# bnbowman/pbccs

Hardware: AMD Instinct MI355X
Metric: CCS ZMWs/sec (and GCUPS) at 1/2/4/8 MI355X vs host-CPU ccs (higher is better)
Workload: dtype f64

## Files before the change

### include/pbccs_amd.h

```cpp
#ifndef PBCCS_AMD_H
#define PBCCS_AMD_H

#ifdef __cplusplus
extern "C" {
#endif

#define PBCCS_OK 0
#define PBCCS_EINVAL (-1)
#define PBCCS_EOOM (-2)
#define PBCCS_EDEVICE (-3)
#define PBCCS_ESTATE (-4)
#define PBCCS_ERANGE (-5)

#define PBCCS_INSERTION 0
#define PBCCS_DELETION 1
#define PBCCS_SUBSTITUTION 2
#define PBCCS_FORWARD_STRAND 0
#define PBCCS_REVERSE_STRAND 1
#define PBCCS_ADD_SUCCESS 0
#define PBCCS_ADD_ALPHABETAMISMATCH 1
#define PBCCS_ADD_MEM_FAIL 2
#define PBCCS_ADD_POOR_ZSCORE 3
#define PBCCS_ADD_OTHER 4
#define PBCCS_ZMW_SUCCESS 0
// ... 118 lines not shown
    long long fill_launches, score_launches, score_tasks, mutations;
    long long band_top_bytes;
    long long band_region_bytes;
    long long band_used_bytes;
    long long pool_mapped_bytes;
    long long oom_retries;
    long long create_host_ns;
    long long create_upload_ns;
    long long derive_ns;
    long long fill_work[16];
    long long scan_reads;
    long long uncertain_reads;
    long long exact_rounds;
    long long uncertain_why[4];
    long long repeat_skipped_ckpt;
} pbccs_counters;
int pbccs_engine_counters(pbccs_engine* eng, pbccs_counters* out, int reset);

typedef struct {
    char name[32];
    long long launches;
    double device_ms;
    double cells;
    double bytes;
    double wave_s;
} pbccs_kernel_stat;
int pbccs_engine_set_profiling(pbccs_engine* eng, int on);
int pbccs_engine_kernel_stats(pbccs_engine* eng, pbccs_kernel_stat* out, int cap, int* n, int reset);


// ... 710 lines not shown
```

### pbccs_amd/csrc/arrow_device.hpp

```cpp
#pragma once

#include <hip/hip_runtime.h>
#include <stdint.h>

namespace pbccs {

constexpr int kCtxZero = 8;
constexpr int kCtxStride = 5;
constexpr int kNoMutation = -100;
constexpr int kMaxExtCols = 4;
constexpr int kMaxFlipFlops = 5;
constexpr double kAlphaBetaTol = 0.001;
constexpr double kRebandFrac = 0.04;

enum MutType : int { kIns = 0, kDel = 1, kSub = 2 };
enum Strand : int { kFwd = 0, kRev = 1 };

enum FillStatus : int { kFillOk = 0, kFillMismatch = 1, kFillOverflow = 2, kFillBadInput = 3, kFillTall = 4,
                        kFillUncertain = 5 };
constexpr double kUnitRoundoff = 0x1p-53;

__host__ __device__ inline int mut_code(int pos, int type, int base) { return (pos << 4) | (type << 2) | base; }
__host__ __device__ inline int mut_pos(int c) { return c >> 4; }
__host__ __device__ inline int mut_type(int c) { return (c >> 2) & 3; }
// ... 23 lines not shown
    const long long* rSeqOff;
    const int* rLen;
    const int* rStrand;
    const int* rTs;
    const int* rTe;
    const int* rActive;
    const int* rZmw;
    const long long* rColBase;
    const long long* rValA;
    const long long* rValB;
    const long long* rValCap;
    const int* rCkpt;
    const char* seqPool;
    int2* aRange;
    int* aOff;
    double* aLs;
    double* aPre;
    int2* bRange;
    int* bOff;
    double* bLs;
    double* bSuf;
    double* valPool;
    double* rBaseline;
    double* rDev;
    int* rFlips;
    int* rStatus;
    double prNot;
    double prThird;
    double sdn;
    unsigned long long* stats;
};

enum StatKind : int { kStatFill = 0, kStatSuffix = 1, kStatScore = 2, kStatFillTall = 3 };
enum WaveSlot : int { kWaveFill = 10, kWaveFillTall = 11, kWaveScore = 12, kWaveSuffix = 13, kWaveReduce = 14 };
#ifndef PBCCS_WAVE_STAMPS
#define PBCCS_WAVE_STAMPS 0
#endif
__device__ __forceinline__ long long wave_t0(const unsigned long long* stats)
{
    if (!PBCCS_WAVE_STAMPS) return 0;
    return stats ? (long long)__builtin_amdgcn_s_memrealtime() : 0;
}
__device__ __forceinline__ void wave_ticks(unsigned long long* stats, int slot, long long t0)
{
    if (!PBCCS_WAVE_STAMPS || !stats) return;
// ... 419 lines not shown
```

### pbccs_amd/csrc/arrow_kernels.hip

```cpp
#include "arrow_device.hpp"
#include "arrow_kernels.hpp"
#include "arrow_score_device.hpp"
#include "coop_chain.hpp"

#include <climits>

namespace pbccs {

__device__ __forceinline__ LaneBand scratch_band(const FillScratch& F, int g, int l, int which)
{
    const long long gm = 2LL * g + which;
    LaneBand m;
    m.range = F.range + gm * F.capCols * 64 + l;
    m.off = F.off + gm * F.capCols * 64 + l;
    m.ls = F.ls + gm * F.capCols * 64 + l;
    m.val = F.val + gm * F.capSlots * 64 + l;
    m.cap = F.capSlots;
    return m;
}

__global__ void __launch_bounds__(64) k_fill(DevBatch B, FillScratch F, const int* __restrict__ reads, int n)
{
    const int t = blockIdx.x * blockDim.x + threadIdx.x;
    if (t >= n) return;
// ... 180 lines not shown
        }
        __syncthreads();
    }
}

constexpr int kSuffixTile = 2048;

__device__ __forceinline__ double add8(double s, const double* __restrict__ t)
{
    double v[8];
#pragma unroll
    for (int i = 0; i < 8; ++i) v[i] = t[i];
#pragma unroll
    for (int i = 0; i < 8; ++i) s = s + v[i];
    return s;
}

__device__ __forceinline__ void k_suffix_body(DevBatch B, const int* __restrict__ reads, int n, int withPrefix)
{
    __shared__ double tile[kSuffixTile];
    const int r = reads[blockIdx.x];
    if (B.rStatus[r] != kFillOk && B.rStatus[r] != kFillMismatch) return;
    const long long cb = B.rColBase[r];
    const int J = window_view(B, r).Length();
    const double* ls = B.bLs + cb;
    double* suf = B.bSuf + cb;
    const int ncol = J + 1;
    const int lane = threadIdx.x & 63;
    const int wbase = threadIdx.x & ~63;
    for (int k0 = 0; k0 <= ncol; k0 += blockDim.x) {
// ... 4 lines not shown
            __syncthreads();
            for (int q = threadIdx.x; q < kSuffixTile && c0 + q < ncol; q += blockDim.x) tile[q] = ls[c0 + q];
            __syncthreads();
            const int hi = min(ncol - c0, kSuffixTile);
            int q = max(kb - c0, 0);
            const int headEnd = min(hi, kb + 64 - c0);
            for (; q < headEnd; ++q) {
                const double v = tile[q];
                if (c0 + q >= k) s = s + v;
            }
            for (; q + 8 <= hi; q += 8) s = add8(s, tile + q);
            for (; q < hi; ++q) s = s + tile[q];
        }
        if (k <= ncol) suf[k] = s;
    }
    if (!withPrefix) return;
    if (threadIdx.x != 0) return;
    const double* als = B.aLs + cb;
    double* pre = B.aPre + cb;
    double run = 0.0;
    pre[0] = 0.0;
    int k = 0;
    for (; k + 8 <= ncol; k += 8) {
        double v[8];
#pragma unroll
        for (int q = 0; q < 8; ++q) v[q] = als[k + q];
#pragma unroll
        for (int q = 0; q < 8; ++q) {
            run = run + v[q];
            pre[k + q + 1] = run;
// ... 74 lines not shown

__device__ __forceinline__ MidGeom middle_geometry(const Band& a, const Band& b, int sc, int bc)
{
    MidGeom g;
    const int2 r0 = a.range[sc - 1], r1 = a.range[sc], r2 = a.range[sc + 1], r3 = a.range[sc + 2];
    g.b0 = min(min(r1.x, r0.x), r2.x);
    g.e0 = max(max(r1.y, r0.y), r2.y);
    g.b1 = min(min(r2.x, r1.x), r3.x);
    g.e1 = max(max(r2.y, r1.y), r3.y);
    const int2 q0 = b.range[bc], q1 = b.range[bc + 1];
    g.lb = min(min(g.b0, g.b1), min(q0.x, q1.x));
    g.le = max(max(g.e0, g.e1), max(q0.y, q1.y));
    return g;
}

__device__ __forceinline__ double score_middle(const ScoreCtx& S, int sc, int bc, const MidGeom& g,
                                               const double* __restrict__ av, int2 ar,
                                               const double* __restrict__ bv, int2 br,
                                               const char* __restrict__ rdp, TaskStat& st)
{
    const int I = S.I;
    char t0, t1, t2, t3;
    int x0, x1, x2, x3;
    S.tv.At(sc - 2, t0, x0);
    S.tv.At(sc - 1, t1, x1);
    S.tv.At(sc, t2, x2);
    S.tv.At(sc + 1, t3, x3);
    (void)t0;
    const double* P0 = S.P.P(sc > 1 ? x0 : kCtxZero);
    const double* P1 = S.P.P(x1);
    const double* P2 = S.P.P(x2);
    const double pM0 = P0[kM], pD0 = P0[kD], cB0 = P1[kB], cS0 = P1[kS3];
    const double pM1 = P1[kM], pD1 = P1[kD], cB1 = P2[kB], cS1 = P2[kS3];
    const double lM = P2[kM], lD = P2[kD];
    const double pn = S.P.prNot, p3 = S.P.prThird;

#define PB_ALPHA(i) (((i) >= ar.x && (i) < ar.y) ? av[(i)] : 0.0)
#define PB_BETA(i) (((i) >= br.x && (i) < br.y) ? bv[-(i)] : 0.0)
#define PB_CELL(out, i, rb, curB, nxtB, pM, pD, cB, cS, pd, pl, rawPrev)                    \
    {                                                                                     \
        const double em_ = ((rb) == (curB)) ? pn : p3;                                    \
        double s_ = ((i) > 0) ? (((i) < I) ? (pd) * (pM) * em_ : 0.0) : (rawPrev);        \
        if ((i) > 1 && (i) < I) s_ = s_ + (rawPrev) * (((nxtB) == (rb)) ? (cB) : (cS));   \
        if ((i) != I) s_ = s_ + (pl) * (pD);                                              \
        out = s_;                                                                         \
    }

    double C0 = 0.0;
    {
        double aD = PB_ALPHA(g.b0 - 1), raw = 0.0;
        for (int i = g.b0; i < g.e0; ++i) {
            const double aL = PB_ALPHA(i);
            const char rb = rdp[i - 1];
            double v;
            PB_CELL(v, i, rb, t1, t2, pM0, pD0, cB0, cS0, aD, aL, raw);
            raw = v;
            if (C0 < v) C0 = v;
            aD = aL;
        }
    }
    const bool s0 = (C0 != 0.0 && C0 != 1.0);
    const int u0 = min(g.b0, g.b1), u1 = max(g.e0, g.e1);
    double C1 = 0.0;
    {
        double aD = PB_ALPHA(u0 - 1), raw0 = 0.0, raw1 = 0.0, sc0p = 0.0;
        for (int i = u0; i < u1; ++i) {
            const double aL = PB_ALPHA(i);
            const char rb = rdp[i - 1];
            double v0 = 0.0, v1 = 0.0, sc0 = 0.0;
            if (i >= g.b0 && i < g.e0) {
                PB_CELL(v0, i, rb, t1, t2, pM0, pD0, cB0, cS0, aD, aL, raw0);
                sc0 = s0 ? v0 / C0 : v0;
            }
            if (i >= g.b1 && i < g.e1) {
                PB_CELL(v1, i, rb, t2, t3, pM1, pD1, cB1, cS1, sc0p, sc0, raw1);
                if (C1 < v1) C1 = v1;
            }
            raw0 = v0;
            raw1 = v1;
            sc0p = sc0;
            aD = aL;
        }
    }
    const bool s1 = (C1 != 0.0 && C1 != 1.0);
    double v = 0.0;
    {
        double aD = PB_ALPHA(g.lb - 1), raw0 = 0.0, raw1 = 0.0, sc0p = 0.0;
        double bH = PB_BETA(g.lb);
        for (int i = g.lb; i < g.le; ++i) {
            const double aL = PB_ALPHA(i);
            const double bN = PB_BETA(i + 1);
            const char rb = (i >= 1) ? rdp[i - 1] : (char)0;
            double v0 = 0.0, v1 = 0.0, sc0 = 0.0, sc1 = 0.0;
            if (i >= g.b0 && i < g.e0) {
                PB_CELL(v0, i, rb, t1, t2, pM0, pD0, cB0, cS0, aD, aL, raw0);
                sc0 = s0 ? v0 / C0 : v0;
            }
            if (i >= g.b1 && i < g.e1) {
                PB_CELL(v1, i, rb, t2, t3, pM1, pD1, cB1, cS1, sc0p, sc0, raw1);
                sc1 = s1 ? v1 / C1 : v1;
            }
            if (i < I) {
                const double mprob = lM * ((rdp[i] == t3) ? pn : p3);
                v = v + sc1 * mprob * bN;
// ... 204 lines not shown
            for (int q = lane; q < spanR; q += 64) ws.rd[q] = gr[q];
            aBase = offLo;
            bBase = boHi;
            rBase = r0;
        }
    }
    __syncthreads();

    TaskStat st;
    double d = 0.0;
    if (scored) {
        if (middle) {
            const int2 ar = S.a.range[sc - 1];
            const int2 br = S.b.range[bc];
            const int ao = S.a.off[sc - 1], bo = S.b.off[bc];
            double score;
            if (staged) {
                const double* av = ws.a + (ao - aBase) - ar.x;
                const double* bv = ws.b + (bo - bBase) + (br.y - 1);
                const char* rdp = ws.rd - rBase;
                score = score_middle(S, sc, bc, g, av, ar, bv, br, rdp, st);
            } else {
                const double* av = S.a.val + ao - ar.x;
                const double* bv = S.b.val + bo + (br.y - 1);
                score = score_middle(S, sc, bc, g, av, ar, bv, br, S.rd, st);
            }
            d = score - B.rBaseline[r];
        } else {
            const int slot = atomicAdd(W.edgeCount, 1);
            if (slot < W.edgeCap) {
                W.edgeList[3 * slot + 0] = k;
                W.edgeList[3 * slot + 1] = rr;
                W.edgeList[3 * slot + 2] = m;
            } else {
                atomicOr(scratch.overflow, 2);
            }
        }
    }
    if (valid && !(scored && !middle)) W.delta[W.deltaBase[k] + (long long)rr * M + m] = d;
    if (B.stats) {
// ... 314 lines not shown
                const double* src = bV + bO[ckB];
                for (int i = lane; i < r0.y - r0.x; i += 64) slot[sOff[nA] + i] = src[i];
                for (int j = ckB - 1; j >= jbLo; --j) {
                    const int2 nr = bR[j + 1], rg = bR[j];
                    __builtin_amdgcn_fence(__ATOMIC_ACQ_REL, "workgroup");
                    replay_beta(X, j, slot + sOff[nA + (ckB - (j + 1))], nr.x, nr.y, slot + sOff[nA + (ckB - j)], rg.x,
                                rg.y);
                }
            }
            __builtin_amdgcn_fence(__ATOMIC_ACQ_REL, "workgroup");
            if (mine) {
                const int2 ar = aR[ja];
                const int2 br = bR[bc];
                const double* av = slot + sOff[ja - ckA] - ar.x;
                const double* bv = slot + sOff[nA + (ckB - bc)] + (br.y - 1);
                const double score = score_middle(S, sc, bc, g, av, ar, bv, br, S.rd, st);
                W.delta[W.deltaBase[k] + (long long)rr * M + m] = score - B.rBaseline[r];
            }
            pending = pending && !mine;
            __syncthreads();
        }
        if (B.stats) {
            unsigned long long c2 = st.cells, b2 = st.bytes;
            for (int w = 32; w > 0; w >>= 1) {
                c2 += __shfl_xor(c2, w, 64);
                b2 += __shfl_xor(b2, w, 64);
            }
            if (lane == 0) {
                atomicAdd(&B.stats[2 * kStatScore], c2);
                atomicAdd(&B.stats[2 * kStatScore + 1], b2);
            }
// ... 325 lines not shown
```

### pbccs_amd/csrc/capi.hip

```cpp
#include "../../include/pbccs_amd.h"

#include <hip/hip_runtime.h>

#include <algorithm>
#include <array>
#include <atomic>
#include <chrono>
#include <cmath>
#include <condition_variable>
#include <cstdio>
#include <cstdlib>
#include <cstring>
#include <functional>
#include <limits>
#include <memory>
#include <mutex>
#include <new>
#include <stdexcept>
#include <string>
#include <thread>
#include <vector>

#include "align_band.hpp"
#include "align_kernels.hpp"
// ... 294 lines not shown
    out->band_region_bytes = eng->counters.bandRegionBytes;
    out->band_used_bytes = eng->counters.bandUsedBytes;
    long long mapped = 0;
    for (const auto& s : eng->slots) mapped += (long long)s->val.mapped_bytes();
    out->pool_mapped_bytes = mapped;
    out->oom_retries = eng->oomRetries;
    out->create_host_ns = eng->createHostNs;
    out->create_upload_ns = eng->createUploadNs;
    out->derive_ns = eng->counters.deriveNs;
    for (int k = 0; k < 16; ++k) out->fill_work[k] = eng->counters.fillWork[k];
    out->scan_reads = eng->counters.scanReads;
    out->uncertain_reads = eng->counters.uncertainReads;
    out->exact_rounds = eng->counters.exactRounds;
    for (int k = 0; k < 4; ++k) out->uncertain_why[k] = eng->counters.uncertainWhy[k];
    out->repeat_skipped_ckpt = eng->repeatSkippedCkpt;
    if (reset) {
        eng->counters = Counters();
        eng->oomRetries = 0;
        eng->repeatSkippedCkpt = 0;
        eng->createHostNs = eng->createUploadNs = 0;
    }
    return PBCCS_OK;
}

int pbccs_scorer_create(pbccs_engine* eng, const pbccs_arrow_config* cfg, const char* tpl, int tpl_len,
                        pbccs_scorer** out)
{
    if (!eng || !cfg || !tpl || tpl_len <= 0 || !out) return fail(PBCCS_EINVAL, "bad argument");
    return guarded([&] {
        std::unique_ptr<pbccs_scorer> s(new pbccs_scorer());
// ... 4 lines not shown
        *out = s.release();
        return PBCCS_OK;
    });
}

void pbccs_scorer_destroy(pbccs_scorer* s) { delete s; }

int pbccs_scorer_add_read(pbccs_scorer* s, const char* seq, int len, int strand, int tstart, int tend,
                          double threshold, int* result)
{
    if (!s || !seq || len < 0 || !result || (strand != 0 && strand != 1)) return fail(PBCCS_EINVAL, "bad argument");
    return guarded([&] {
        ArrowBatch& B = *s->batch;
        const int r = B.AppendRead(s->z, std::string(seq, len), strand, tstart, tend);
        B.FillReads({r});
        *result = B.FinishAddRead(r, threshold);
        return PBCCS_OK;
    });
}

int pbccs_scorer_score_many(pbccs_scorer* s, const pbccs_mutation* m, int n, double fast_threshold, double* scores)
{
    if (!s || (n > 0 && (!m || !scores)) || n < 0) return fail(PBCCS_EINVAL, "bad argument");
    return guarded([&] {
        ArrowBatch& B = *s->batch;
        const int L = (int)B.Template(s->z).size();
        std::vector<std::vector<int>> codes(1);
        for (int i = 0; i < n; ++i) {
            Mutation mu;
            if (!to_mutation(m[i], L, &mu)) return fail(PBCCS_EINVAL, "invalid single-base mutation");
// ... 207 lines not shown
static void merge_engine_stats(pbccs_engine* eng, ArrowBatch& B)
{
    std::lock_guard<std::mutex> lk(eng->statsMu);
    try {
        const Counters& c = B.counters();
        eng->counters.fillLaunches += c.fillLaunches;
        eng->counters.scoreLaunches += c.scoreLaunches;
        eng->counters.scoreTasks += c.scoreTasks;
        eng->counters.mutations += c.mutations;
        eng->counters.deriveNs += c.deriveNs;
        eng->counters.scanReads += c.scanReads;
        eng->counters.uncertainReads += c.uncertainReads;
        eng->counters.exactRounds += c.exactRounds;
        for (int k = 0; k < 4; ++k) eng->counters.uncertainWhy[k] += c.uncertainWhy[k];
        for (int k = 0; k < 16; ++k) eng->counters.fillWork[k] += c.fillWork[k];
        eng->counters.bandTopBytes = std::max(eng->counters.bandTopBytes, c.bandTopBytes);
        eng->counters.bandRegionBytes = std::max(eng->counters.bandRegionBytes, c.bandRegionBytes);
        eng->counters.bandUsedBytes = std::max(eng->counters.bandUsedBytes, c.bandUsedBytes);
        B.ResetCounters();
        B.CollectProfile(eng->stats);
    } catch (...) {
        (void)hipGetLastError();
    }
}

static int create_batch(pbccs_engine* eng, const pbccs_zmw_input* in, int n, const pbccs_polish_options* opts,
                        int slot, pbccs_batch** out, const pbccs_repeat_options* repeats = nullptr)
{
    if (!eng || n < 0 || (n > 0 && !in) || !out) return fail(PBCCS_EINVAL, "bad argument");
    return guarded([&] {
// ... 4286 lines not shown
```

### pbccs_amd/csrc/engine.hip

```cpp
#include "engine.hpp"
#include "diploid_kernels.hpp"
#include "refine_repeats.hpp"
#include "strand_kernels.hpp"

#include <hipcub/hipcub.hpp>

#include <algorithm>
#include <mutex>
#include <climits>
#include <cmath>
#include <cstdio>
#include <cstdlib>
#include <cstring>
#include <numeric>
#include <set>
#include <stdexcept>
#include <chrono>
#include <unordered_set>

namespace pbccs {

#define PBCCS_HIP(x)                                                         \
    do {                                                                     \
        hipError_t e_ = (x);                                                 \
// ... 316 lines not shown
{
    if (stream) (void)hipStreamSynchronize(stream);
    if (stream2) (void)hipStreamSynchronize(stream2);
    for (hipEvent_t e : eventPool) (void)hipEventDestroy(e);
    if (evFork) (void)hipEventDestroy(evFork);
    if (evJoin) (void)hipEventDestroy(evJoin);
    if (stream2) (void)hipStreamDestroy(stream2);
    if (stream) (void)hipStreamDestroy(stream);
}

size_t Workspace::TrimRetired()
{
    size_t b = 0;
    auto t = [&](auto& v) { b += v.trim(); };
    t(hDesc);
    t(selBase); t(nSel); t(colScratch); t(bump); t(desc); t(seq); t(ckPairs); t(ckStart); t(rBaseline); t(rFlips);
    t(rDev); t(wDev); t(wAmb);
    t(rStatus); t(usedA); t(usedB); t(maxH); t(wZmw); t(wNMut); t(wMutBase); t(wDeltaBase); t(wWaveStart);
    t(wMutStart); t(wPosStart); t(wPosBase); t(wQvBase); t(stats); t(aRange); t(bRange); t(aOff); t(bOff); t(aLs);
    t(bLs); t(aPre); t(bSuf); t(fVal); t(fLs); t(fPre); t(fRange); t(fOff); t(codes); t(posOff); t(qv); t(list);
    t(edge); t(edgeCount); t(ckSlots); t(ckCounter); t(delta); t(score); t(fav); t(scratch); t(scratchTop);
    t(scratchOverflow); t(xStage); t(sel); t(selCount); t(selScore); t(selCode); t(selRank); t(selTmp);
    b += val.trim_fallback();
    return b;
}

void Workspace::EnsureStreams()
{
    if (stream) return;
    PBCCS_HIP(hipStreamCreateWithFlags(&stream, hipStreamNonBlocking));
    PBCCS_HIP(hipStreamCreateWithFlags(&stream2, hipStreamNonBlocking));
    PBCCS_HIP(hipEventCreateWithFlags(&evFork, hipEventDisableTiming));
    PBCCS_HIP(hipEventCreateWithFlags(&evJoin, hipEventDisableTiming));
}

ArrowBatch::ArrowBatch(int device, Workspace* shared, bool ownStreams, bool wsBuffers)
    : device_(device),
      ownWs_(shared ? nullptr : new Workspace()),
      ws_(shared ? shared : ownWs_.get()),
      dSelBase_(ws_->selBase), dNSel_(ws_->nSel), dColScratch_(ws_->colScratch), dBump_(ws_->bump),
      hDesc_(ws_->hDesc), dCkPairs_(ws_->ckPairs), dCkStart_(ws_->ckStart), dRBaseline_(ws_->rBaseline),
      dRDev_(ws_->rDev),
      dRFlips_(ws_->rFlips), dRStatus_(ws_->rStatus), dUsedA_(ws_->usedA), dUsedB_(ws_->usedB), dMaxH_(ws_->maxH),
      dWZmw_(ws_->wZmw), dWNMut_(ws_->wNMut), dWMutBase_(ws_->wMutBase), dWDeltaBase_(ws_->wDeltaBase),
      dWWaveStart_(ws_->wWaveStart), dWMutStart_(ws_->wMutStart), dWPosStart_(ws_->wPosStart),
      dWPosBase_(ws_->wPosBase), dWQvBase_(ws_->wQvBase),
      dARange_(ws_->aRange), dBRange_(ws_->bRange), dAOff_(ws_->aOff), dBOff_(ws_->bOff), dALs_(ws_->aLs),
      dBLs_(ws_->bLs), dAPre_(ws_->aPre), dBSuf_(ws_->bSuf), dVal_(ws_->val), dCodes_(ws_->codes),
      dPosOff_(ws_->posOff), dQv_(ws_->qv), dList_(ws_->list), dEdge_(ws_->edge), dEdgeCount_(ws_->edgeCount),
      dDelta_(ws_->delta), dScore_(ws_->score), dFav_(ws_->fav), dScratch_(ws_->scratch),
      dScratchTop_(ws_->scratchTop), dScratchOverflow_(ws_->scratchOverflow), dStats_(ws_->stats),
      eventPool_(ws_->eventPool), dDesc_(wsBuffers && shared ? ws_->desc : ownDesc_),
      dSeq_(wsBuffers && shared ? ws_->seq : ownSeq_)
{
    PBCCS_HIP(hipSetDevice(device_));
    if (const char* e = std::getenv("PBCCS_INITIAL_BAND_HEIGHT")) initialBandHeight_ = std::max(1, std::atoi(e));
    ckpt_policy(&ckptK_, &ckptMinLen_);
    ckptAll_ = std::min(kCkptMaxK, std::max(0, env_int("PBCCS_CKPT_ALL", 0)));
    if (ownStreams) {
        ownStreams_ = true;
        PBCCS_HIP(hipStreamCreateWithFlags(&stream_, hipStreamNonBlocking));
        static const bool oneStream = env_int("PBCCS_ONE_STREAM", 0) != 0;
        if (oneStream) stream2_ = stream_;
        else PBCCS_HIP(hipStreamCreateWithFlags(&stream2_, hipStreamNonBlocking));
        PBCCS_HIP(hipEventCreateWithFlags(&evFork_, hipEventDisableTiming));
        PBCCS_HIP(hipEventCreateWithFlags(&evJoin_, hipEventDisableTiming));
    } else {
        ws_->EnsureStreams();
        stream_ = ws_->stream;
        stream2_ = ws_->stream2;
        evFork_ = ws_->evFork;
        evJoin_ = ws_->evJoin;
    }
// ... 138 lines not shown
        out[k].ms += stats_[k].ms;
        out[k].cells += stats_[k].cells;
        out[k].bytes += stats_[k].bytes;
        out[k].waveTicks += stats_[k].waveTicks;
        stats_[k] = KernelStat();
    }
}

void ArrowBatch::Prepare()
{
    const StreamScope bound(stream_);
    const size_t cols = std::max<long long>(colTop_, 1);
    dARange_.reserve(cols, false);
    dBRange_.reserve(cols, false);
    dAOff_.reserve(cols, false);
    dBOff_.reserve(cols, false);
    dALs_.reserve(cols, false);
    dBLs_.reserve(cols, false);
    dAPre_.reserve(cols, false);
    dBSuf_.reserve(cols, false);
    dVal_.reserve(std::max<long long>(valTop_, 1), false);
    UploadReads();
    long long mut = 0, delta = 0, pos = 0;
    for (const HZmw& z : zmws_) {
        const long long M = unique_mutation_count(z.tpl) + 64;
        mut += M;
        delta += M * z.nReads;
        pos += (long long)z.tpl.size() + 65;
    }
    dCodes_.reserve(std::max<long long>(mut, 1), false);
// ... 272 lines not shown
    pRValB_ = reinterpret_cast<long long*>(base + oVb);
    pRValCap_ = reinterpret_cast<long long*>(base + oVc);
    pRLen_ = reinterpret_cast<int*>(base + oRl);
    pRStrand_ = reinterpret_cast<int*>(base + oRs);
    pRTs_ = reinterpret_cast<int*>(base + oRts);
    pRTe_ = reinterpret_cast<int*>(base + oRte);
    pRActive_ = reinterpret_cast<int*>(base + oRa);
    pRZmw_ = reinterpret_cast<int*>(base + oRz);
    pRCkpt_ = reinterpret_cast<int*>(base + oRck);
    pTpl_ = base + oTpl;
    UploadReads();
    const size_t cols = std::max<long long>(colTop_, 1);
    dARange_.reserve(cols, true);
    dBRange_.reserve(cols, true);
    dAOff_.reserve(cols, true);
    dBOff_.reserve(cols, true);
    dALs_.reserve(cols, true);
    dBLs_.reserve(cols, true);
    dAPre_.reserve(cols, true);
    dBSuf_.reserve(cols, true);
    dVal_.reserve(std::max<long long>(valTop_, 1), true);
    dRBaseline_.reserve(std::max(R, 1), true);
    dRDev_.reserve(std::max(R, 1), true);
    dRFlips_.reserve(std::max(R, 1), true);
    dRStatus_.reserve(std::max(R, 1), true);
    PBCCS_HIP(hipStreamSynchronize(stream_));
    descDirty_ = false;
}

DevBatch ArrowBatch::View() const
// ... 24 lines not shown
    b.aLs = dALs_.ptr;
    b.aPre = dAPre_.ptr;
    b.bRange = dBRange_.ptr;
    b.bOff = dBOff_.ptr;
    b.bLs = dBLs_.ptr;
    b.bSuf = dBSuf_.ptr;
    b.valPool = dVal_.ptr;
    b.rBaseline = dRBaseline_.ptr;
    b.rDev = dRDev_.ptr;
    b.rFlips = dRFlips_.ptr;
    b.rStatus = dRStatus_.ptr;
    b.prNot = 1.0 - kMismatchProbability;
    b.prThird = kMismatchProbability / 3.0;
    b.sdn = zmws_.empty() ? std::exp(12.5) : std::exp(zmws_[0].opt.scoreDiff);
    b.stats = profiling_ ? dStats_.ptr : nullptr;
    return b;
}

void ArrowBatch::FillReads(const std::vector<int>& readsIn)
{
    const StreamScope bound(stream_);
    constexpr int kPaths = 4;
    for (int r : readsIn) EnsureCapacity(r);
    auto promote = [&](int r, int p) {
        HRead& h = reads_[r];
        int q = p + 1;
        if (q == 2 && (long long)h.seq.size() + 1 > 4LL * kCoopTallRows) q = 3;
        h.fillPath = q;
        if (q >= 2 && q < kPaths) {
            const long long I = (long long)h.seq.size(), J = h.te - h.ts;
// ... 101 lines not shown
        int nScan[kPaths] = {};
        for (int p = 2; p < kPaths; ++p) {
            if (!((scanPaths >> (p - 2)) & 1)) continue;
            std::stable_partition(todo[p].begin(), todo[p].end(), scannable);
            nScan[p] = (int)std::count_if(todo[p].begin(), todo[p].end(), scannable);
        }
        const bool anyScan = nScan[2] + nScan[3] > 0;
        UploadDescriptors();
        const size_t R = reads_.size();
        dUsedA_.reserve(std::max<size_t>(R, 1), true);
        dUsedB_.reserve(std::max<size_t>(R, 1), true);
        dMaxH_.reserve(std::max<size_t>(R, 1), true);
        std::vector<int> list;
        for (auto& v : todo) list.insert(list.end(), v.begin(), v.end());
        upload(dList_, list, stream_);
        const DevBatch B = View();
        size_t off = 0;
        const bool forked = !todo[2].empty() || !todo[3].empty();
        const auto tLaunch = std::chrono::steady_clock::now();
        const bool grow = ws_->val.allowVmm;
        long long headroom = 0;
        if (grow) {
            long long want = 1ll << 24;
            for (int p = 2; p < kPaths; ++p)
                for (int r : todo[p]) {
                    const long long I = (long long)reads_[r].seq.size(), J = reads_[r].te - reads_[r].ts;
                    const long long K = std::max(1, reads_[r].ckpt);
                    want += 2 * std::max<long long>(0, (I + 1) * (J + 1) / 7 / K - reads_[r].valCap);
                }
            size_t freeB = 0, totalB = 0;
            PBCCS_HIP(hipMemGetInfo(&freeB, &totalB));
            static const long long margin = (long long)env_int("PBCCS_HEADROOM_MARGIN_GB", (int)(kHeadroomMargin >> 30)) << 30;
            const long long spare = std::max<long long>(0, (long long)freeB - margin);
            headroom = std::min<long long>(want, spare / 4 / (long long)sizeof(double));
            dVal_.reserve((size_t)std::max<long long>(valTop_, 1), true);
            dVal_.try_reserve((size_t)std::max<long long>(valTop_ + headroom, 1));
            dBump_.reserve(1, false);
            const unsigned long long top = (unsigned long long)valTop_;
            PBCCS_HIP(hipMemcpyAsync(dBump_.ptr, &top, sizeof(top), hipMemcpyHostToDevice, stream_));
        }
        const long long valLimit = grow ? (long long)dVal_.cap : 0;
        if (forked) {
            PBCCS_HIP(hipEventRecord(evFork_, stream_));
            PBCCS_HIP(hipStreamWaitEvent(stream2_, evFork_, 0));
        }
        for (int p = 0; p < kPaths; ++p) {
            const int n = (int)todo[p].size();
            if (n == 0) continue;
            int maxI = 1, maxJ = 1;
            for (int r : todo[p]) {
                maxI = std::max(maxI, (int)reads_[r].seq.size());
                maxJ = std::max(maxJ, reads_[r].te - reads_[r].ts);
// ... 159 lines not shown
                h.status = st[r];
                h.flips = fl[r];
                h.baseline = bl[r];
                h.dev = !dv.empty() ? dv[r] : 0.0;
                h.filled = true;
                h.usedA = ua[r];
                h.usedB = ub[r];
                if (p >= 1) h.maxH = mh[r];
                if (st[r] == kFillOk || st[r] == kFillMismatch) done.push_back(r);
            }
        }
        for (int p = 0; p < kPaths; ++p) todo[p].swap(next[p]);
    }
    if (!done.empty()) {
        upload(dList_, done, stream_);
        const DevBatch B = View();
        Timed(kKSuffix, [&] { launch_suffix(B, dList_.ptr, (int)done.size(), stream_, true); });
        PBCCS_HIP(hipGetLastError());
        PBCCS_HIP(hipStreamSynchronize(stream_));
    }
    if (!serial.empty()) FillReadsSerial(serial);
    (void)counters();
}

void ArrowBatch::FillReadsSerial(const std::vector<int>& readsIn)
{
    const StreamScope bound(stream_);
    std::vector<int> todo(readsIn);
    for (int r : todo)
        if (reads_[r].ckpt != 0) {
            reads_[r].ckpt = 0;
            descDirty_ = true;
        }
    for (int r : todo) EnsureCapacity(r);
// ... 61 lines not shown
                h.filled = true;
                h.usedA = ua[r];
                h.usedB = ub[r];
                if (st[r] == kFillOk || st[r] == kFillMismatch) {
                    const long long need = std::max(ua[r], ub[r]);
                    if (need > h.valCap) {
                        h.valCap = need + need / 4 + 64;
                        h.valA = valTop_;
                        h.valB = valTop_ + h.valCap;
                        valTop_ += 2 * h.valCap;
                        descDirty_ = true;
                    }
                }
            }
            UploadDescriptors();
            const DevBatch B2 = View();
            Timed(kKCompact, [&] { launch_compact(B2, F, dList_.ptr, (int)n, stream_); });
            Timed(kKSuffix, [&] { launch_suffix(B2, dList_.ptr, (int)n, stream_); });
            PBCCS_HIP(hipGetLastError());
            PBCCS_HIP(hipStreamSynchronize(stream_));
            pos += n;
        }
        todo.swap(again);
        H *= 2;
    }
}

void ArrowBatch::TraceSummary(size_t n, int H, long long capSlots)
{
    std::vector<long long> tr;
    download(tr, dTrace_, 8 * n, stream_);
    PBCCS_HIP(hipStreamSynchronize(stream_));
    long long t0 = LLONG_MAX, t1 = 0, maxDur = 0, maxCells = 0, sumCells = 0, sumPass = 0, maxPass = 0;
    double sumDur = 0;
    long long done = 0;
// ... 1247 lines not shown
```

### pbccs_amd/csrc/engine.hpp

```cpp
#pragma once

#include <hip/hip_runtime.h>

#include <algorithm>
#include <cstdint>
#include <limits>
#include <memory>
#include <string>
#include <utility>
#include <vector>

#include "arrow_device.hpp"
#include "arrow_kernels.hpp"
#include "arrow_model.hpp"

namespace pbccs {

struct ArrowOptions {
    double scoreDiff = 12.5;
    double fastScoreThreshold = -12.5;
    double addThreshold = std::numeric_limits<double>::quiet_NaN();
};

struct RefineOptions {
// ... 172 lines not shown
    std::vector<size_t> sizes_;
    DevVec<double> fallback_;
};

struct Counters {
    long long fillCells = 0, fillLaunches = 0;
    long long scoreTasks = 0, scoreLaunches = 0;
    long long mutations = 0;
    long long bandGrowths = 0;
    long long relayouts = 0;
    long long bandTopBytes = 0, bandRegionBytes = 0, bandUsedBytes = 0;
    long long deriveNs = 0;
    long long scanReads = 0, uncertainReads = 0, exactRounds = 0;
    long long uncertainWhy[4] = {};
    long long fillWork[16] = {};
};

void ckpt_policy(int* K, int* minLen);

enum KernelKind {
    kKFill = 0, kKSuffix, kKEnumerate, kKScore, kKReduce, kKQv, kKSelect, kKCompact, kKFillTall,
    kKQFillGrp, kKQFillCoop, kKQFillLane, kKQScoreMid, kKQScoreMulti, kKScoreWide, kKQvRich, kKStrandSums,
    kKStrandSites, kKernelKinds
};
extern const char* const kKernelNames[kKernelKinds];

struct StrandOptions {
    double minScore = 12.5;
    int minReads = 2;
};
// ... 30 lines not shown
    DevVec<double> colScratch;
    DevVec<unsigned long long> bump;
    PinnedBuf hDesc;
    DevVec<char> desc, seq;
    DevVec<int2> ckPairs;
    DevVec<long long> ckStart;
    DevVec<double> rBaseline, rDev;
    DevVec<double> wDev;
    DevVec<int> wAmb;
    DevVec<int> rFlips, rStatus, usedA, usedB, maxH;
    DevVec<int> wZmw, wNMut;
    DevVec<long long> wMutBase, wDeltaBase, wWaveStart, wMutStart, wPosStart, wPosBase, wQvBase;
    DevVec<unsigned long long> stats;
    DevVec<int2> aRange, bRange;
    DevVec<int> aOff, bOff;
    DevVec<double> aLs, bLs, aPre, bSuf;
    VmPool val;
    DevVec<double> fVal, fLs, fPre;
    DevVec<int2> fRange;
    DevVec<int> fOff;
    DevVec<int> codes, posOff, qv, list, edge, edgeCount;
    DevVec<double> ckSlots;
    DevVec<unsigned long long> ckCounter;
    DevVec<double> delta, score;
    DevVec<unsigned char> fav;
    DevVec<double> scratch;
    DevVec<unsigned long long> scratchTop;
    DevVec<int> scratchOverflow;
    DevVec<unsigned char> xStage;
    DevVec<long long> sel, selCount;
// ... 47 lines not shown
    int NumReads(int z) const { return zmws_[z].nReads; }
    int ReadIndex(int z, int k) const { return zmws_[z].readBegin + k; }
    const std::string& Template(int z) const { return zmws_[z].tpl; }
    std::string TemplateRev(int z) const { return reverse_complement(zmws_[z].tpl); }
    double ReadScore(int r) const { return reads_[r].baseline; }
    bool ReadActive(int r) const { return reads_[r].active; }
    int ReadTs(int r) const { return reads_[r].ts; }
    int ReadTe(int r) const { return reads_[r].te; }
    int ReadStrand(int r) const { return reads_[r].strand; }
    int ReadFlips(int r) const { return reads_[r].flips; }
    double BaselineScore(int z) const;
    void ZScores(int z, double* zg, double* za, std::vector<double>* zs) const;
    const ArrowOptions& Options(int z) const { return zmws_[z].opt; }
    const Counters& counters();
    void ResetCounters() { counters_ = Counters(); }
    hipStream_t stream() const { return stream_; }
    void Prepare();
    void SetProfiling(bool on);
    void CollectProfile(KernelStat out[kKernelKinds]);

private:
    struct HZmw {
        std::string tpl;
        double snr[4];
        bool derived = false;
        double ctx[45];
        TransParams trans[8];
        double ctxMeanVar[9][2];
        ArrowOptions opt;
        int readBegin = 0, nReads = 0;
// ... 39 lines not shown
                  bool needPositions, bool phased = false);

    int device_ = 0;
    std::unique_ptr<Workspace> ownWs_;
    Workspace* ws_;
    hipStream_t stream_ = nullptr;
    bool ownStreams_ = false;
    hipStream_t stream2_ = nullptr;
    hipEvent_t evFork_ = nullptr, evJoin_ = nullptr;
    DevVec<long long>& dSelBase_;
    DevVec<int>& dNSel_;
    DevVec<double>& dColScratch_;
    DevVec<long long> dCoopTrace_[4];
    DevVec<unsigned long long> dFillWork_;
    DevVec<unsigned long long>& dBump_;
    std::vector<HZmw> zmws_;
    std::vector<HRead> reads_;
    long long tplTop_ = 0, seqTop_ = 0, colTop_ = 0, valTop_ = 0;
    int initialBandHeight_ = 16;
    bool descDirty_ = true;
    bool reclaim_ = false;
    size_t seqUploaded_ = 0;

    std::vector<char> hTpl_, hSeq_;
    std::vector<unsigned char> hXStage_;
    DevVec<char> ownDesc_, ownSeq_;
    DevVec<char>& dDesc_;
    DevVec<char>& dSeq_;
    PinnedBuf& hDesc_;
    int *pZFwd_ = nullptr, *pZRev_ = nullptr, *pZLen_ = nullptr, *pZReadBegin_ = nullptr, *pZNReads_ = nullptr;
// ... 4 lines not shown
        *pRZmw_ = nullptr, *pRCkpt_ = nullptr;
    DevVec<int2>& dCkPairs_;
    DevVec<long long>& dCkStart_;
    int ckptK_ = 0, ckptMinLen_ = 0, ckptAll_ = 0;
    long long ckSlotCap_ = 0;
    DevVec<double>& dRBaseline_;
    DevVec<double>& dRDev_;
    bool scan_ = false;
    DevVec<int>& dRFlips_, &dRStatus_, &dUsedA_, &dUsedB_, &dMaxH_;
    DevVec<int>& dWZmw_, &dWNMut_;
    DevVec<long long>& dWMutBase_, &dWDeltaBase_, &dWWaveStart_, &dWMutStart_, &dWPosStart_, &dWPosBase_,
        &dWQvBase_;
    DevVec<int2>& dARange_;
    DevVec<int2>& dBRange_;
    DevVec<int>& dAOff_;
    DevVec<int>& dBOff_;
    DevVec<double>& dALs_;
    DevVec<double>& dBLs_;
    DevVec<double>& dAPre_;
    DevVec<double>& dBSuf_;
    VmPool& dVal_;
    DevVec<int>& dCodes_;
    DevVec<int>& dPosOff_;
    DevVec<int>& dQv_;
    DevVec<int>& dList_;
    DevVec<int>& dEdge_;
    DevVec<int>& dEdgeCount_;
    DevVec<double>& dDelta_;
    DevVec<double>& dScore_;
    DevVec<unsigned char>& dFav_;
// ... 31 lines not shown
```

### pbccs_amd/lib.py

```python
import ctypes
import os

HERE = os.path.dirname(os.path.abspath(__file__))
LIB_PATH = os.environ.get("PBCCS_LIB") or os.path.join(HERE, "_lib", "libpbccs_amd.so")

PBCCS_OK = 0
ERRORS = {-1: "EINVAL", -2: "EOOM", -3: "EDEVICE", -4: "ESTATE", -5: "ERANGE"}

_lib = None


class PbccsError(RuntimeError):
    def __init__(self, code, msg):
        super().__init__(f"pbccs {ERRORS.get(code, code)}: {msg}")
        self.code = code


class CMutation(ctypes.Structure):
    _fields_ = [("type", ctypes.c_int), ("start", ctypes.c_int), ("end", ctypes.c_int), ("new_base", ctypes.c_char)]


class CMutationEx(ctypes.Structure):
    _fields_ = [("type", ctypes.c_int), ("start", ctypes.c_int), ("end", ctypes.c_int),
                ("new_bases", ctypes.c_char_p), ("n_bases", ctypes.c_int)]
# ... 40 lines not shown

class CKernelStat(ctypes.Structure):
    _fields_ = [("name", ctypes.c_char * 32), ("launches", ctypes.c_longlong), ("device_ms", ctypes.c_double),
                ("cells", ctypes.c_double), ("bytes", ctypes.c_double), ("wave_s", ctypes.c_double)]


class CCounters(ctypes.Structure):
    _fields_ = [("fill_launches", ctypes.c_longlong), ("score_launches", ctypes.c_longlong),
                ("score_tasks", ctypes.c_longlong), ("mutations", ctypes.c_longlong),
                ("band_top_bytes", ctypes.c_longlong), ("band_region_bytes", ctypes.c_longlong),
                ("band_used_bytes", ctypes.c_longlong), ("pool_mapped_bytes", ctypes.c_longlong),
                ("oom_retries", ctypes.c_longlong), ("create_host_ns", ctypes.c_longlong),
                ("create_upload_ns", ctypes.c_longlong), ("derive_ns", ctypes.c_longlong),
                ("fill_work", ctypes.c_longlong * 16), ("scan_reads", ctypes.c_longlong),
                ("uncertain_reads", ctypes.c_longlong), ("exact_rounds", ctypes.c_longlong),
                ("uncertain_why", ctypes.c_longlong * 4), ("repeat_skipped_ckpt", ctypes.c_longlong)]


class CQvModelParams(ctypes.Structure):
    _fields_ = [(n, ctypes.c_float) for n in ("match", "mismatch", "mismatch_s", "branch", "branch_s", "deletion_n",
                                              "deletion_with_tag", "deletion_with_tag_s", "nce", "nce_s")] + \
               [("merge", ctypes.c_float * 4), ("merge_s", ctypes.c_float * 4)]


class CQuiverConfig(ctypes.Structure):
    _fields_ = [("params", CQvModelParams), ("moves_available", ctypes.c_int), ("score_diff", ctypes.c_float),
                ("fast_score_threshold", ctypes.c_float), ("add_threshold", ctypes.c_float),
                ("sum_product", ctypes.c_int), ("recursor", ctypes.c_int)]


class CQuiverRead(ctypes.Structure):
# ... 530 lines not shown
```

Measured before the change: 3609.

## Trim leading zero alpha rows from mutation scoring via per-column nonzero edge

During the suffix pass, each alpha column is scanned for its first nonzero band entry and that row is stored in a new per-column array. The mutation scoring kernel then starts its middle-column loops at that row instead of the band start, skipping rows that contribute only zeros. The feature is on by default behind an environment flag and is bypassed for checkpointed reads. The extra suffix-kernel scan, the new device array, and the counter readback and memset add work and host synchronization.

```diff
diff --git a/include/pbccs_amd.h b/include/pbccs_amd.h
--- a/include/pbccs_amd.h
+++ b/include/pbccs_amd.h
@@ -156,6 +156,7 @@
     long long exact_rounds;
     long long uncertain_why[4];
     long long repeat_skipped_ckpt;
+    long long zero_edge_rows;
 } pbccs_counters;
 int pbccs_engine_counters(pbccs_engine* eng, pbccs_counters* out, int reset);
 
diff --git a/pbccs_amd/csrc/arrow_device.hpp b/pbccs_amd/csrc/arrow_device.hpp
--- a/pbccs_amd/csrc/arrow_device.hpp
+++ b/pbccs_amd/csrc/arrow_device.hpp
@@ -61,6 +61,7 @@
     const char* seqPool;
     int2* aRange;
     int* aOff;
+    int* aNz;
     double* aLs;
     double* aPre;
     int2* bRange;
@@ -76,6 +77,8 @@
     double prThird;
     double sdn;
     unsigned long long* stats;
+    int zeroEdges;
+    unsigned long long* zeroEdgeRows;
 };
 
 enum StatKind : int { kStatFill = 0, kStatSuffix = 1, kStatScore = 2, kStatFillTall = 3 };
diff --git a/pbccs_amd/csrc/arrow_kernels.hip b/pbccs_amd/csrc/arrow_kernels.hip
--- a/pbccs_amd/csrc/arrow_kernels.hip
+++ b/pbccs_amd/csrc/arrow_kernels.hip
@@ -218,6 +218,78 @@
 #pragma unroll
     for (int i = 0; i < 8; ++i) s = s + v[i];
     return s;
+}
+
+constexpr int kEdgeCols = 4;
+
+__device__ __forceinline__ void zero_edges(const DevBatch& B, int r, long long cb, int ncol)
+{
+    __shared__ unsigned long long waveRows[4];
+    const int2* __restrict__ rng = B.aRange + cb;
+    const int* __restrict__ off = B.aOff + cb;
+    int* __restrict__ nz = B.aNz + cb;
+    const int lane = threadIdx.x & 63;
+    const int wv = threadIdx.x >> 6;
+    if (!B.zeroEdges || (B.rCkpt && B.rCkpt[r] != 0)) {
+        for (int c = threadIdx.x; c < ncol; c += blockDim.x) nz[c] = rng[c].x;
+        return;
+    }
+    const double* __restrict__ val = B.valPool + B.rValA[r];
+    unsigned long long rows = 0;
+    for (int c0 = wv * 64; c0 < ncol; c0 += blockDim.x) {
+        const int c = c0 + lane;
+        int2 rg = make_int2(0, 0);
+        int o = 0;
+        if (c < ncol) {
+            rg = rng[c];
+            o = off[c];
+        }
+        int mine = rg.x;
+        const bool zero0 = c < ncol && rg.x < rg.y && val[o] == 0.0;
+        unsigned long long todo = __ballot(zero0);
+        while (todo != 0) {
+            int q[kEdgeCols], bx[kEdgeCols], by[kEdgeCols], bo[kEdgeCols];
+            double v[kEdgeCols];
+#pragma unroll
+            for (int u = 0; u < kEdgeCols; ++u) {
+                q[u] = __builtin_amdgcn_readfirstlane(todo != 0 ? __ffsll((long long)todo) - 1 : -1);
+                todo &= todo - (todo != 0 ? 1ull : 0ull);
+                const int ql = max(q[u], 0);
+                bx[u] = __builtin_amdgcn_readlane(rg.x, ql);
+                by[u] = q[u] >= 0 ? __builtin_amdgcn_readlane(rg.y, ql) : bx[u];
+                bo[u] = __builtin_amdgcn_readlane(o, ql);
+                v[u] = (bx[u] + lane < by[u]) ? val[bo[u] + lane] : 0.0;
+            }
+#pragma unroll
+            for (int u = 0; u < kEdgeCols; ++u) {
+                unsigned long long m = __ballot(v[u] != 0.0);
+                int e = by[u];
+                if (m != 0) e = bx[u] + (__ffsll((long long)m) - 1);
+                else
+                    for (int i0 = bx[u] + 64; i0 < by[u]; i0 += 64) {
+                        const int i = i0 + lane;
+                        const double w = (i < by[u]) ? val[bo[u] + (i - bx[u])] : 0.0;
+                        m = __ballot(w != 0.0);
+                        if (m != 0) {
+                            e = i0 + (__ffsll((long long)m) - 1);
+                            break;
+                        }
+                    }
+                if (lane == q[u]) mine = e;
+            }
+        }
+        if (c < ncol) {
+            nz[c] = mine;
+            rows += (unsigned long long)max(0, mine - rg.x);
+        }
+    }
+    for (int q = 32; q > 0; q >>= 1) rows += __shfl_xor(rows, q, 64);
+    if (lane == 0) waveRows[wv] = rows;
+    __syncthreads();
+    if (threadIdx.x == 0 && B.zeroEdgeRows) {
+        const unsigned long long sum = waveRows[0] + waveRows[1] + waveRows[2] + waveRows[3];
+        if (sum != 0) atomicAdd(B.zeroEdgeRows, sum);
+    }
 }
 
 __device__ __forceinline__ void k_suffix_body(DevBatch B, const int* __restrict__ reads, int n, int withPrefix)
@@ -252,6 +324,7 @@
         }
         if (k <= ncol) suf[k] = s;
     }
+    zero_edges(B, r, cb, ncol);
     if (!withPrefix) return;
     if (threadIdx.x != 0) return;
     const double* als = B.aLs + cb;
@@ -356,10 +429,12 @@
     return g;
 }
 
+template <bool kTrim>
 __device__ __forceinline__ double score_middle(const ScoreCtx& S, int sc, int bc, const MidGeom& g,
                                                const double* __restrict__ av, int2 ar,
                                                const double* __restrict__ bv, int2 br,
-                                               const char* __restrict__ rdp, TaskStat& st)
+                                               const char* __restrict__ rdp, TaskStat& st, int z = 0,
+                                               bool trim3 = false)
 {
     const int I = S.I;
     char t0, t1, t2, t3;
@@ -390,8 +465,9 @@
 
     double C0 = 0.0;
     {
-        double aD = PB_ALPHA(g.b0 - 1), raw = 0.0;
-        for (int i = g.b0; i < g.e0; ++i) {
+        const int f0 = kTrim ? z : g.b0;
+        double aD = PB_ALPHA(f0 - 1), raw = 0.0;
+        for (int i = f0; i < g.e0; ++i) {
             const double aL = PB_ALPHA(i);
             const char rb = rdp[i - 1];
             double v;
@@ -402,7 +478,7 @@
         }
     }
     const bool s0 = (C0 != 0.0 && C0 != 1.0);
-    const int u0 = min(g.b0, g.b1), u1 = max(g.e0, g.e1);
+    const int u0 = kTrim ? z : min(g.b0, g.b1), u1 = max(g.e0, g.e1);
     double C1 = 0.0;
     {
         double aD = PB_ALPHA(u0 - 1), raw0 = 0.0, raw1 = 0.0, sc0p = 0.0;
@@ -427,9 +503,10 @@
     const bool s1 = (C1 != 0.0 && C1 != 1.0);
     double v = 0.0;
     {
-        double aD = PB_ALPHA(g.lb - 1), raw0 = 0.0, raw1 = 0.0, sc0p = 0.0;
-        double bH = PB_BETA(g.lb);
-        for (int i = g.lb; i < g.le; ++i) {
+        const int l0 = (kTrim && trim3) ? u0 : g.lb, l1 = (kTrim && trim3) ? g.e1 : g.le;
+        double aD = PB_ALPHA(l0 - 1), raw0 = 0.0, raw1 = 0.0, sc0p = 0.0;
+        double bH = PB_BETA(l0);
+        for (int i = l0; i < l1; ++i) {
             const double aL = PB_ALPHA(i);
             const double bN = PB_BETA(i + 1);
             const char rb = (i >= 1) ? rdp[i - 1] : (char)0;
@@ -664,16 +741,18 @@
             const int2 ar = S.a.range[sc - 1];
             const int2 br = S.b.range[bc];
             const int ao = S.a.off[sc - 1], bo = S.b.off[bc];
+            const int nz = B.aNz[B.rColBase[r] + (sc - 1)];
+            const bool trim = B.zeroEdges != 0;
             double score;
             if (staged) {
                 const double* av = ws.a + (ao - aBase) - ar.x;
                 const double* bv = ws.b + (bo - bBase) + (br.y - 1);
                 const char* rdp = ws.rd - rBase;
-                score = score_middle(S, sc, bc, g, av, ar, bv, br, rdp, st);
+                score = score_middle<true>(S, sc, bc, g, av, ar, bv, br, rdp, st, nz, trim);
             } else {
                 const double* av = S.a.val + ao - ar.x;
                 const double* bv = S.b.val + bo + (br.y - 1);
-                score = score_middle(S, sc, bc, g, av, ar, bv, br, S.rd, st);
+                score = score_middle<true>(S, sc, bc, g, av, ar, bv, br, S.rd, st, nz, trim);
             }
             d = score - B.rBaseline[r];
         } else {
@@ -1018,7 +1097,7 @@
                 const int2 br = bR[bc];
                 const double* av = slot + sOff[ja - ckA] - ar.x;
                 const double* bv = slot + sOff[nA + (ckB - bc)] + (br.y - 1);
-                const double score = score_middle(S, sc, bc, g, av, ar, bv, br, S.rd, st);
+                const double score = score_middle<false>(S, sc, bc, g, av, ar, bv, br, S.rd, st);
                 W.delta[W.deltaBase[k] + (long long)rr * M + m] = score - B.rBaseline[r];
             }
             pending = pending && !mine;
diff --git a/pbccs_amd/csrc/capi.hip b/pbccs_amd/csrc/capi.hip
--- a/pbccs_amd/csrc/capi.hip
+++ b/pbccs_amd/csrc/capi.hip
@@ -332,6 +332,7 @@
     out->exact_rounds = eng->counters.exactRounds;
     for (int k = 0; k < 4; ++k) out->uncertain_why[k] = eng->counters.uncertainWhy[k];
     out->repeat_skipped_ckpt = eng->repeatSkippedCkpt;
+    out->zero_edge_rows = eng->counters.zeroEdgeRows;
     if (reset) {
         eng->counters = Counters();
         eng->oomRetries = 0;
@@ -366,6 +367,10 @@
         ArrowBatch& B = *s->batch;
         const int r = B.AppendRead(s->z, std::string(seq, len), strand, tstart, tend);
         B.FillReads({r});
+        {
+            std::lock_guard<std::mutex> lk(s->eng->statsMu);
+            s->eng->counters.zeroEdgeRows += B.TakeZeroEdgeRows();
+        }
         *result = B.FinishAddRead(r, threshold);
         return PBCCS_OK;
     });
@@ -603,6 +608,7 @@
         eng->counters.exactRounds += c.exactRounds;
         for (int k = 0; k < 4; ++k) eng->counters.uncertainWhy[k] += c.uncertainWhy[k];
         for (int k = 0; k < 16; ++k) eng->counters.fillWork[k] += c.fillWork[k];
+        eng->counters.zeroEdgeRows += c.zeroEdgeRows;
         eng->counters.bandTopBytes = std::max(eng->counters.bandTopBytes, c.bandTopBytes);
         eng->counters.bandRegionBytes = std::max(eng->counters.bandRegionBytes, c.bandRegionBytes);
         eng->counters.bandUsedBytes = std::max(eng->counters.bandUsedBytes, c.bandUsedBytes);
diff --git a/pbccs_amd/csrc/engine.hip b/pbccs_amd/csrc/engine.hip
--- a/pbccs_amd/csrc/engine.hip
+++ b/pbccs_amd/csrc/engine.hip
@@ -354,7 +354,7 @@
     size_t b = 0;
     auto t = [&](auto& v) { b += v.trim(); };
     t(hDesc);
-    t(selBase); t(nSel); t(colScratch); t(bump); t(desc); t(seq); t(ckPairs); t(ckStart); t(rBaseline); t(rFlips);
+    t(selBase); t(nSel); t(colScratch); t(bump); t(aNz); t(desc); t(seq); t(ckPairs); t(ckStart); t(rBaseline); t(rFlips);
     t(rDev); t(wDev); t(wAmb);
     t(rStatus); t(usedA); t(usedB); t(maxH); t(wZmw); t(wNMut); t(wMutBase); t(wDeltaBase); t(wWaveStart);
     t(wMutStart); t(wPosStart); t(wPosBase); t(wQvBase); t(stats); t(aRange); t(bRange); t(aOff); t(bOff); t(aLs);
@@ -385,8 +385,8 @@
       dWZmw_(ws_->wZmw), dWNMut_(ws_->wNMut), dWMutBase_(ws_->wMutBase), dWDeltaBase_(ws_->wDeltaBase),
       dWWaveStart_(ws_->wWaveStart), dWMutStart_(ws_->wMutStart), dWPosStart_(ws_->wPosStart),
       dWPosBase_(ws_->wPosBase), dWQvBase_(ws_->wQvBase),
-      dARange_(ws_->aRange), dBRange_(ws_->bRange), dAOff_(ws_->aOff), dBOff_(ws_->bOff), dALs_(ws_->aLs),
-      dBLs_(ws_->bLs), dAPre_(ws_->aPre), dBSuf_(ws_->bSuf), dVal_(ws_->val), dCodes_(ws_->codes),
+      dARange_(ws_->aRange), dBRange_(ws_->bRange), dAOff_(ws_->aOff), dANz_(ws_->aNz), dBOff_(ws_->bOff),
+      dALs_(ws_->aLs), dBLs_(ws_->bLs), dAPre_(ws_->aPre), dBSuf_(ws_->bSuf), dVal_(ws_->val), dCodes_(ws_->codes),
       dPosOff_(ws_->posOff), dQv_(ws_->qv), dList_(ws_->list), dEdge_(ws_->edge), dEdgeCount_(ws_->edgeCount),
       dDelta_(ws_->delta), dScore_(ws_->score), dFav_(ws_->fav), dScratch_(ws_->scratch),
       dScratchTop_(ws_->scratchTop), dScratchOverflow_(ws_->scratchOverflow), dStats_(ws_->stats),
@@ -397,6 +397,7 @@
     if (const char* e = std::getenv("PBCCS_INITIAL_BAND_HEIGHT")) initialBandHeight_ = std::max(1, std::atoi(e));
     ckpt_policy(&ckptK_, &ckptMinLen_);
     ckptAll_ = std::min(kCkptMaxK, std::max(0, env_int("PBCCS_CKPT_ALL", 0)));
+    zeroEdges_ = env_int("PBCCS_SCORE_ZERO_EDGES", 1) != 0;
     if (ownStreams) {
         ownStreams_ = true;
         PBCCS_HIP(hipStreamCreateWithFlags(&stream_, hipStreamNonBlocking));
@@ -565,6 +566,7 @@
     dARange_.reserve(cols, false);
     dBRange_.reserve(cols, false);
     dAOff_.reserve(cols, false);
+    dANz_.reserve(cols, false);
     dBOff_.reserve(cols, false);
     dALs_.reserve(cols, false);
     dBLs_.reserve(cols, false);
@@ -867,6 +869,7 @@
     dARange_.reserve(cols, true);
     dBRange_.reserve(cols, true);
     dAOff_.reserve(cols, true);
+    dANz_.reserve(cols, true);
     dBOff_.reserve(cols, true);
     dALs_.reserve(cols, true);
     dBLs_.reserve(cols, true);
@@ -921,6 +924,9 @@
     b.prThird = kMismatchProbability / 3.0;
     b.sdn = zmws_.empty() ? std::exp(12.5) : std::exp(zmws_[0].opt.scoreDiff);
     b.stats = profiling_ ? dStats_.ptr : nullptr;
+    b.aNz = dANz_.ptr;
+    b.zeroEdges = zeroEdges_ ? 1 : 0;
+    b.zeroEdgeRows = dBump_.ptr ? dBump_.ptr + 1 : nullptr;
     return b;
 }
 
@@ -1052,6 +1058,7 @@
         std::vector<int> list;
         for (auto& v : todo) list.insert(list.end(), v.begin(), v.end());
         upload(dList_, list, stream_);
+        dBump_.reserve(2, false);
         const DevBatch B = View();
         size_t off = 0;
         const bool forked = !todo[2].empty() || !todo[3].empty();
@@ -1073,7 +1080,6 @@
             headroom = std::min<long long>(want, spare / 4 / (long long)sizeof(double));
             dVal_.reserve((size_t)std::max<long long>(valTop_, 1), true);
             dVal_.try_reserve((size_t)std::max<long long>(valTop_ + headroom, 1));
-            dBump_.reserve(1, false);
             const unsigned long long top = (unsigned long long)valTop_;
             PBCCS_HIP(hipMemcpyAsync(dBump_.ptr, &top, sizeof(top), hipMemcpyHostToDevice, stream_));
         }
@@ -1263,10 +1269,14 @@
     }
     if (!done.empty()) {
         upload(dList_, done, stream_);
+        PBCCS_HIP(hipMemsetAsync(dBump_.ptr + 1, 0, sizeof(unsigned long long), stream_));
         const DevBatch B = View();
         Timed(kKSuffix, [&] { launch_suffix(B, dList_.ptr, (int)done.size(), stream_, true); });
         PBCCS_HIP(hipGetLastError());
+        unsigned long long zeroRows = 0;
+        d2h(&zeroRows, dBump_.ptr + 1, sizeof(zeroRows), stream_);
         PBCCS_HIP(hipStreamSynchronize(stream_));
+        counters_.zeroEdgeRows += (long long)zeroRows;
     }
     if (!serial.empty()) FillReadsSerial(serial);
     (void)counters();
@@ -1358,11 +1368,16 @@
                 }
             }
             UploadDescriptors();
+            dBump_.reserve(2, false);
+            PBCCS_HIP(hipMemsetAsync(dBump_.ptr + 1, 0, sizeof(unsigned long long), stream_));
             const DevBatch B2 = View();
             Timed(kKCompact, [&] { launch_compact(B2, F, dList_.ptr, (int)n, stream_); });
             Timed(kKSuffix, [&] { launch_suffix(B2, dList_.ptr, (int)n, stream_); });
             PBCCS_HIP(hipGetLastError());
+            unsigned long long zeroRows = 0;
+            d2h(&zeroRows, dBump_.ptr + 1, sizeof(zeroRows), stream_);
             PBCCS_HIP(hipStreamSynchronize(stream_));
+            counters_.zeroEdgeRows += (long long)zeroRows;
             pos += n;
         }
         todo.swap(again);
diff --git a/pbccs_amd/csrc/engine.hpp b/pbccs_amd/csrc/engine.hpp
--- a/pbccs_amd/csrc/engine.hpp
+++ b/pbccs_amd/csrc/engine.hpp
@@ -210,6 +210,7 @@
     long long scanReads = 0, uncertainReads = 0, exactRounds = 0;
     long long uncertainWhy[4] = {};
     long long fillWork[16] = {};
+    long long zeroEdgeRows = 0;
 };
 
 void ckpt_policy(int* K, int* minLen);
@@ -270,6 +271,7 @@
     DevVec<unsigned long long> stats;
     DevVec<int2> aRange, bRange;
     DevVec<int> aOff, bOff;
+    DevVec<int> aNz;
     DevVec<double> aLs, bLs, aPre, bSuf;
     VmPool val;
     DevVec<double> fVal, fLs, fPre;
@@ -347,6 +349,12 @@
     const ArrowOptions& Options(int z) const { return zmws_[z].opt; }
     const Counters& counters();
     void ResetCounters() { counters_ = Counters(); }
+    long long TakeZeroEdgeRows()
+    {
+        const long long n = counters_.zeroEdgeRows;
+        counters_.zeroEdgeRows = 0;
+        return n;
+    }
     hipStream_t stream() const { return stream_; }
     void Prepare();
     void SetProfiling(bool on);
@@ -416,6 +424,7 @@
     DevVec<long long> dCoopTrace_[4];
     DevVec<unsigned long long> dFillWork_;
     DevVec<unsigned long long>& dBump_;
+    bool zeroEdges_ = true;
     std::vector<HZmw> zmws_;
     std::vector<HRead> reads_;
     long long tplTop_ = 0, seqTop_ = 0, colTop_ = 0, valTop_ = 0;
@@ -450,6 +459,7 @@
     DevVec<int2>& dARange_;
     DevVec<int2>& dBRange_;
     DevVec<int>& dAOff_;
+    DevVec<int>& dANz_;
     DevVec<int>& dBOff_;
     DevVec<double>& dALs_;
     DevVec<double>& dBLs_;
diff --git a/pbccs_amd/lib.py b/pbccs_amd/lib.py
--- a/pbccs_amd/lib.py
+++ b/pbccs_amd/lib.py
@@ -78,7 +78,8 @@
                 ("create_upload_ns", ctypes.c_longlong), ("derive_ns", ctypes.c_longlong),
                 ("fill_work", ctypes.c_longlong * 16), ("scan_reads", ctypes.c_longlong),
                 ("uncertain_reads", ctypes.c_longlong), ("exact_rounds", ctypes.c_longlong),
-                ("uncertain_why", ctypes.c_longlong * 4), ("repeat_skipped_ckpt", ctypes.c_longlong)]
+                ("uncertain_why", ctypes.c_longlong * 4), ("repeat_skipped_ckpt", ctypes.c_longlong),
+                ("zero_edge_rows", ctypes.c_longlong)]
 
 
 class CQvModelParams(ctypes.Structure):
```

New measurement: 3569. 0.989x the previous value.
